# facebookresearch/co-tracker

Hardware: NVIDIA H100
Metric: tracked points*frames/sec at N=6400, T=16, 512^2 (higher is better)
Workload: dtype transformer + corr_mlp.fc2 + input_transform: bf16x3; correlation einsum: fp16x2; corr_mlp.fc1: bf16x3; fp32 accumulate, fp32 softmax/LayerNorm/GELU

## Files before the change

cotracker_b200/csrc/common.cuh:

```cuda
#pragma once
#include <cuda.h>
#include <cuda_bf16.h>
#include <cuda_fp16.h>
#include <cuda_runtime.h>
#include <stdint.h>

#include <atomic>

namespace ct3 {

struct DeviceOnce { std::atomic<uint64_t> done[2] = {}; };
template <typename F>
inline cudaError_t once_per_device(DeviceOnce& flag, F&& f) {
  int dev = 0;
  cudaError_t e = cudaGetDevice(&dev);
  if (e != cudaSuccess) return e;
  if (dev < 0 || dev >= 128) return f();
  const uint64_t bit = 1ull << (dev & 63);
  if (flag.done[dev >> 6].load(std::memory_order_acquire) & bit) return cudaSuccess;
  e = f();
  if (e == cudaSuccess) flag.done[dev >> 6].fetch_or(bit, std::memory_order_release);
  return e;
}

// ... 148 lines not shown
__device__ __forceinline__ uint8_t* smem_align1024(uint8_t* raw) {
  return raw + ((1024u - (smem_u32(raw) & 1023u)) & 1023u);
}

__device__ __forceinline__ void tma_prefetch_desc(const CUtensorMap* m) {
  asm volatile("prefetch.tensormap [%0];" ::"l"(reinterpret_cast<uint64_t>(m)) : "memory");
}
__device__ __forceinline__ void tma_load_2d(void* smem_dst, const CUtensorMap* m, int c0, int c1,
                                            uint64_t* bar) {
  asm volatile(
      "cp.async.bulk.tensor.2d.shared::cluster.global.mbarrier::complete_tx::bytes [%0], [%1, {%3, %4}], [%2];"
      ::"r"(smem_u32(smem_dst)), "l"(reinterpret_cast<uint64_t>(m)), "r"(smem_u32(bar)), "r"(c0), "r"(c1)
      : "memory");
}

__device__ __forceinline__ void tma_load_4d(void* smem_dst, const CUtensorMap* m, int c0, int c1, int c2, int c3,
                                            uint64_t* bar) {
  asm volatile(
      "cp.async.bulk.tensor.4d.shared::cluster.global.mbarrier::complete_tx::bytes [%0], [%1, {%3, %4, %5, %6}], [%2];"
      ::"r"(smem_u32(smem_dst)), "l"(reinterpret_cast<uint64_t>(m)), "r"(smem_u32(bar)), "r"(c0), "r"(c1), "r"(c2),
      "r"(c3)
      : "memory");
}

__device__ __forceinline__ uint64_t l2_policy_evict_first() {
  uint64_t p;
  asm volatile("createpolicy.fractional.L2::evict_first.b64 %0, 1.0;" : "=l"(p));
  return p;
}
__device__ __forceinline__ uint64_t l2_policy_evict_last() {
  uint64_t p;
  asm volatile("createpolicy.fractional.L2::evict_last.b64 %0, 1.0;" : "=l"(p));
  return p;
}
__device__ __forceinline__ void tma_load_4d_hint(void* smem_dst, const CUtensorMap* m, int c0, int c1, int c2, int c3,
                                                 uint64_t* bar, uint64_t policy) {
  asm volatile(
      "cp.async.bulk.tensor.4d.shared::cluster.global.mbarrier::complete_tx::bytes.L2::cache_hint [%0], [%1, {%3, %4, %5, %6}], [%2], %7;"
      ::"r"(smem_u32(smem_dst)), "l"(reinterpret_cast<uint64_t>(m)), "r"(smem_u32(bar)), "r"(c0), "r"(c1), "r"(c2),
      "r"(c3), "l"(policy)
      : "memory");
}
__device__ __forceinline__ void tma_load_3d(void* smem_dst, const CUtensorMap* m, int c0, int c1, int c2, uint64_t* bar) {
  asm volatile(
      "cp.async.bulk.tensor.3d.shared::cluster.global.mbarrier::complete_tx::bytes [%0], [%1, {%3, %4, %5}], [%2];"
      ::"r"(smem_u32(smem_dst)), "l"(reinterpret_cast<uint64_t>(m)), "r"(smem_u32(bar)), "r"(c0), "r"(c1), "r"(c2)
      : "memory");
}
__device__ __forceinline__ void tma_store_3d(const CUtensorMap* m, int c0, int c1, int c2, const void* smem_src) {
  asm volatile("cp.async.bulk.tensor.3d.global.shared::cta.bulk_group [%0, {%2, %3, %4}], [%1];"
               ::"l"(reinterpret_cast<uint64_t>(m)), "r"(smem_u32(smem_src)), "r"(c0), "r"(c1), "r"(c2)
               : "memory");
}

__device__ __forceinline__ void bulk_store_s2g(void* gdst, const void* ssrc, uint32_t bytes) {
  asm volatile("cp.async.bulk.global.shared::cta.bulk_group [%0], [%1], %2;" ::"l"(gdst), "r"(smem_u32(ssrc)), "r"(bytes)
               : "memory");
}
__device__ __forceinline__ void bulk_store_s2g_hint(void* gdst, const void* ssrc, uint32_t bytes, uint64_t policy) {
  asm volatile("cp.async.bulk.global.shared::cta.bulk_group.L2::cache_hint [%0], [%1], %2, %3;" ::"l"(gdst),
               "r"(smem_u32(ssrc)), "r"(bytes), "l"(policy)
               : "memory");
}
__device__ __forceinline__ void bulk_commit() { asm volatile("cp.async.bulk.commit_group;" ::: "memory"); }
__device__ __forceinline__ void bulk_wait_read0() { asm volatile("cp.async.bulk.wait_group.read 0;" ::: "memory"); }
__device__ __forceinline__ void bulk_wait0() { asm volatile("cp.async.bulk.wait_group 0;" ::: "memory"); }

__device__ __forceinline__ uint64_t gmma_desc_sw128(uint32_t smem_addr) {
  uint64_t d = 0;
  d |= (uint64_t)((smem_addr & 0x3FFFFu) >> 4);
  d |= (uint64_t)1 << 16;
  d |= (uint64_t)(1024 >> 4) << 32;
  d |= (uint64_t)1 << 62;
  return d;
}
__device__ __forceinline__ void wgmma_fence() { asm volatile("wgmma.fence.sync.aligned;" ::: "memory"); }
__device__ __forceinline__ void wgmma_commit() { asm volatile("wgmma.commit_group.sync.aligned;" ::: "memory"); }
template <int R>
__device__ __forceinline__ void wgmma_wait0(float (&d)[R]) {
  asm volatile("wgmma.wait_group.sync.aligned 0;" ::: "memory");
#pragma unroll
  for (int i = 0; i < R; ++i) asm volatile("" : "+f"(d[i])::"memory");
}

__device__ __forceinline__ void wgmma_m64n64_bf16(float (&d)[32], uint64_t da, uint64_t db, uint32_t scale_d) {
  asm volatile(
      "{\n\t.reg .pred p;\n\tsetp.ne.b32 p, %34, 0;\n\t"
      "wgmma.mma_async.sync.aligned.m64n64k16.f32.bf16.bf16 "
      "{%0, %1, %2, %3, %4, %5, %6, %7, %8, %9, %10, %11, %12, %13, %14, %15, %16, %17, %18, %19, %20, %21, %22, %23, %24, %25, %26, %27, %28, %29, %30, %31}, %32, %33, p, 1, 1, 0, 0;\n\t}"
      : "+f"(d[0]), "+f"(d[1]), "+f"(d[2]), "+f"(d[3]), "+f"(d[4]), "+f"(d[5]), "+f"(d[6]), "+f"(d[7]), "+f"(d[8]), "+f"(d[9]), "+f"(d[10]), "+f"(d[11]), "+f"(d[12]), "+f"(d[13]), "+f"(d[14]), "+f"(d[15]), "+f"(d[16]), "+f"(d[17]), "+f"(d[18]), "+f"(d[19]), "+f"(d[20]), "+f"(d[21]), "+f"(d[22]), "+f"(d[23]), "+f"(d[24]), "+f"(d[25]), "+f"(d[26]), "+f"(d[27]), "+f"(d[28]), "+f"(d[29]), "+f"(d[30]), "+f"(d[31])
      : "l"(da), "l"(db), "r"(scale_d));
}
__device__ __forceinline__ void wgmma_m64n128_bf16(float (&d)[64], uint64_t da, uint64_t db, uint32_t scale_d) {
  asm volatile(
      "{\n\t.reg .pred p;\n\tsetp.ne.b32 p, %66, 0;\n\t"
      "wgmma.mma_async.sync.aligned.m64n128k16.f32.bf16.bf16 "
      "{%0, %1, %2, %3, %4, %5, %6, %7, %8, %9, %10, %11, %12, %13, %14, %15, %16, %17, %18, %19, %20, %21, %22, %23, %24, %25, %26, %27, %28, %29, %30, %31, %32, %33, %34, %35, %36, %37, %38, %39, %40, %41, %42, %43, %44, %45, %46, %47, %48, %49, %50, %51, %52, %53, %54, %55, %56, %57, %58, %59, %60, %61, %62, %63}, %64, %65, p, 1, 1, 0, 0;\n\t}"
      : "+f"(d[0]), "+f"(d[1]), "+f"(d[2]), "+f"(d[3]), "+f"(d[4]), "+f"(d[5]), "+f"(d[6]), "+f"(d[7]), "+f"(d[8]), "+f"(d[9]), "+f"(d[10]), "+f"(d[11]), "+f"(d[12]), "+f"(d[13]), "+f"(d[14]), "+f"(d[15]), "+f"(d[16]), "+f"(d[17]), "+f"(d[18]), "+f"(d[19]), "+f"(d[20]), "+f"(d[21]), "+f"(d[22]), "+f"(d[23]), "+f"(d[24]), "+f"(d[25]), "+f"(d[26]), "+f"(d[27]), "+f"(d[28]), "+f"(d[29]), "+f"(d[30]), "+f"(d[31]), "+f"(d[32]), "+f"(d[33]), "+f"(d[34]), "+f"(d[35]), "+f"(d[36]), "+f"(d[37]), "+f"(d[38]), "+f"(d[39]), "+f"(d[40]), "+f"(d[41]), "+f"(d[42]), "+f"(d[43]), "+f"(d[44]), "+f"(d[45]), "+f"(d[46]), "+f"(d[47]), "+f"(d[48]), "+f"(d[49]), "+f"(d[50]), "+f"(d[51]), "+f"(d[52]), "+f"(d[53]), "+f"(d[54]), "+f"(d[55]), "+f"(d[56]), "+f"(d[57]), "+f"(d[58]), "+f"(d[59]), "+f"(d[60]), "+f"(d[61]), "+f"(d[62]), "+f"(d[63])
      : "l"(da), "l"(db), "r"(scale_d));
}
__device__ __forceinline__ void wgmma_m64n144_bf16(float (&d)[72], uint64_t da, uint64_t db, uint32_t scale_d) {
  asm volatile(
      "{\n\t.reg .pred p;\n\tsetp.ne.b32 p, %74, 0;\n\t"
      "wgmma.mma_async.sync.aligned.m64n144k16.f32.bf16.bf16 "
      "{%0, %1, %2, %3, %4, %5, %6, %7, %8, %9, %10, %11, %12, %13, %14, %15, %16, %17, %18, %19, %20, %21, %22, %23, %24, %25, %26, %27, %28, %29, %30, %31, %32, %33, %34, %35, %36, %37, %38, %39, %40, %41, %42, %43, %44, %45, %46, %47, %48, %49, %50, %51, %52, %53, %54, %55, %56, %57, %58, %59, %60, %61, %62, %63, %64, %65, %66, %67, %68, %69, %70, %71}, %72, %73, p, 1, 1, 0, 0;\n\t}"
      : "+f"(d[0]), "+f"(d[1]), "+f"(d[2]), "+f"(d[3]), "+f"(d[4]), "+f"(d[5]), "+f"(d[6]), "+f"(d[7]), "+f"(d[8]), "+f"(d[9]), "+f"(d[10]), "+f"(d[11]), "+f"(d[12]), "+f"(d[13]), "+f"(d[14]), "+f"(d[15]), "+f"(d[16]), "+f"(d[17]), "+f"(d[18]), "+f"(d[19]), "+f"(d[20]), "+f"(d[21]), "+f"(d[22]), "+f"(d[23]), "+f"(d[24]), "+f"(d[25]), "+f"(d[26]), "+f"(d[27]), "+f"(d[28]), "+f"(d[29]), "+f"(d[30]), "+f"(d[31]), "+f"(d[32]), "+f"(d[33]), "+f"(d[34]), "+f"(d[35]), "+f"(d[36]), "+f"(d[37]), "+f"(d[38]), "+f"(d[39]), "+f"(d[40]), "+f"(d[41]), "+f"(d[42]), "+f"(d[43]), "+f"(d[44]), "+f"(d[45]), "+f"(d[46]), "+f"(d[47]), "+f"(d[48]), "+f"(d[49]), "+f"(d[50]), "+f"(d[51]), "+f"(d[52]), "+f"(d[53]), "+f"(d[54]), "+f"(d[55]), "+f"(d[56]), "+f"(d[57]), "+f"(d[58]), "+f"(d[59]), "+f"(d[60]), "+f"(d[61]), "+f"(d[62]), "+f"(d[63]), "+f"(d[64]), "+f"(d[65]), "+f"(d[66]), "+f"(d[67]), "+f"(d[68]), "+f"(d[69]), "+f"(d[70]), "+f"(d[71])
      : "l"(da), "l"(db), "r"(scale_d));
}
__device__ __forceinline__ void wgmma_m64n64_f16(float (&d)[32], uint64_t da, uint64_t db, uint32_t scale_d) {
  asm volatile(
      "{\n\t.reg .pred p;\n\tsetp.ne.b32 p, %34, 0;\n\t"
      "wgmma.mma_async.sync.aligned.m64n64k16.f32.f16.f16 "
      "{%0, %1, %2, %3, %4, %5, %6, %7, %8, %9, %10, %11, %12, %13, %14, %15, %16, %17, %18, %19, %20, %21, %22, %23, %24, %25, %26, %27, %28, %29, %30, %31}, %32, %33, p, 1, 1, 0, 0;\n\t}"
      : "+f"(d[0]), "+f"(d[1]), "+f"(d[2]), "+f"(d[3]), "+f"(d[4]), "+f"(d[5]), "+f"(d[6]), "+f"(d[7]), "+f"(d[8]), "+f"(d[9]), "+f"(d[10]), "+f"(d[11]), "+f"(d[12]), "+f"(d[13]), "+f"(d[14]), "+f"(d[15]), "+f"(d[16]), "+f"(d[17]), "+f"(d[18]), "+f"(d[19]), "+f"(d[20]), "+f"(d[21]), "+f"(d[22]), "+f"(d[23]), "+f"(d[24]), "+f"(d[25]), "+f"(d[26]), "+f"(d[27]), "+f"(d[28]), "+f"(d[29]), "+f"(d[30]), "+f"(d[31])
      : "l"(da), "l"(db), "r"(scale_d));
}
__device__ __forceinline__ void wgmma_m64n128_f16(float (&d)[64], uint64_t da, uint64_t db, uint32_t scale_d) {
  asm volatile(
      "{\n\t.reg .pred p;\n\tsetp.ne.b32 p, %66, 0;\n\t"
      "wgmma.mma_async.sync.aligned.m64n128k16.f32.f16.f16 "
      "{%0, %1, %2, %3, %4, %5, %6, %7, %8, %9, %10, %11, %12, %13, %14, %15, %16, %17, %18, %19, %20, %21, %22, %23, %24, %25, %26, %27, %28, %29, %30, %31, %32, %33, %34, %35, %36, %37, %38, %39, %40, %41, %42, %43, %44, %45, %46, %47, %48, %49, %50, %51, %52, %53, %54, %55, %56, %57, %58, %59, %60, %61, %62, %63}, %64, %65, p, 1, 1, 0, 0;\n\t}"
      : "+f"(d[0]), "+f"(d[1]), "+f"(d[2]), "+f"(d[3]), "+f"(d[4]), "+f"(d[5]), "+f"(d[6]), "+f"(d[7]), "+f"(d[8]), "+f"(d[9]), "+f"(d[10]), "+f"(d[11]), "+f"(d[12]), "+f"(d[13]), "+f"(d[14]), "+f"(d[15]), "+f"(d[16]), "+f"(d[17]), "+f"(d[18]), "+f"(d[19]), "+f"(d[20]), "+f"(d[21]), "+f"(d[22]), "+f"(d[23]), "+f"(d[24]), "+f"(d[25]), "+f"(d[26]), "+f"(d[27]), "+f"(d[28]), "+f"(d[29]), "+f"(d[30]), "+f"(d[31]), "+f"(d[32]), "+f"(d[33]), "+f"(d[34]), "+f"(d[35]), "+f"(d[36]), "+f"(d[37]), "+f"(d[38]), "+f"(d[39]), "+f"(d[40]), "+f"(d[41]), "+f"(d[42]), "+f"(d[43]), "+f"(d[44]), "+f"(d[45]), "+f"(d[46]), "+f"(d[47]), "+f"(d[48]), "+f"(d[49]), "+f"(d[50]), "+f"(d[51]), "+f"(d[52]), "+f"(d[53]), "+f"(d[54]), "+f"(d[55]), "+f"(d[56]), "+f"(d[57]), "+f"(d[58]), "+f"(d[59]), "+f"(d[60]), "+f"(d[61]), "+f"(d[62]), "+f"(d[63])
      : "l"(da), "l"(db), "r"(scale_d));
}
__device__ __forceinline__ void wgmma_m64n144_f16(float (&d)[72], uint64_t da, uint64_t db, uint32_t scale_d) {
  asm volatile(
      "{\n\t.reg .pred p;\n\tsetp.ne.b32 p, %74, 0;\n\t"
      "wgmma.mma_async.sync.aligned.m64n144k16.f32.f16.f16 "
      "{%0, %1, %2, %3, %4, %5, %6, %7, %8, %9, %10, %11, %12, %13, %14, %15, %16, %17, %18, %19, %20, %21, %22, %23, %24, %25, %26, %27, %28, %29, %30, %31, %32, %33, %34, %35, %36, %37, %38, %39, %40, %41, %42, %43, %44, %45, %46, %47, %48, %49, %50, %51, %52, %53, %54, %55, %56, %57, %58, %59, %60, %61, %62, %63, %64, %65, %66, %67, %68, %69, %70, %71}, %72, %73, p, 1, 1, 0, 0;\n\t}"
      : "+f"(d[0]), "+f"(d[1]), "+f"(d[2]), "+f"(d[3]), "+f"(d[4]), "+f"(d[5]), "+f"(d[6]), "+f"(d[7]), "+f"(d[8]), "+f"(d[9]), "+f"(d[10]), "+f"(d[11]), "+f"(d[12]), "+f"(d[13]), "+f"(d[14]), "+f"(d[15]), "+f"(d[16]), "+f"(d[17]), "+f"(d[18]), "+f"(d[19]), "+f"(d[20]), "+f"(d[21]), "+f"(d[22]), "+f"(d[23]), "+f"(d[24]), "+f"(d[25]), "+f"(d[26]), "+f"(d[27]), "+f"(d[28]), "+f"(d[29]), "+f"(d[30]), "+f"(d[31]), "+f"(d[32]), "+f"(d[33]), "+f"(d[34]), "+f"(d[35]), "+f"(d[36]), "+f"(d[37]), "+f"(d[38]), "+f"(d[39]), "+f"(d[40]), "+f"(d[41]), "+f"(d[42]), "+f"(d[43]), "+f"(d[44]), "+f"(d[45]), "+f"(d[46]), "+f"(d[47]), "+f"(d[48]), "+f"(d[49]), "+f"(d[50]), "+f"(d[51]), "+f"(d[52]), "+f"(d[53]), "+f"(d[54]), "+f"(d[55]), "+f"(d[56]), "+f"(d[57]), "+f"(d[58]), "+f"(d[59]), "+f"(d[60]), "+f"(d[61]), "+f"(d[62]), "+f"(d[63]), "+f"(d[64]), "+f"(d[65]), "+f"(d[66]), "+f"(d[67]), "+f"(d[68]), "+f"(d[69]), "+f"(d[70]), "+f"(d[71])
      : "l"(da), "l"(db), "r"(scale_d));
}

__device__ __forceinline__ void wgmma_m64n48_bf16(float (&d)[24], uint64_t da, uint64_t db, uint32_t scale_d) {
  asm volatile(
      "{\n\t.reg .pred p;\n\tsetp.ne.b32 p, %26, 0;\n\t"
      "wgmma.mma_async.sync.aligned.m64n48k16.f32.bf16.bf16 "
      "{%0, %1, %2, %3, %4, %5, %6, %7, %8, %9, %10, %11, %12, %13, %14, %15, %16, %17, %18, %19, %20, %21, %22, %23}, %24, %25, p, 1, 1, 0, 0;\n\t}"
      : "+f"(d[0]), "+f"(d[1]), "+f"(d[2]), "+f"(d[3]), "+f"(d[4]), "+f"(d[5]), "+f"(d[6]), "+f"(d[7]), "+f"(d[8]), "+f"(d[9]), "+f"(d[10]), "+f"(d[11]), "+f"(d[12]), "+f"(d[13]), "+f"(d[14]), "+f"(d[15]), "+f"(d[16]), "+f"(d[17]), "+f"(d[18]), "+f"(d[19]), "+f"(d[20]), "+f"(d[21]), "+f"(d[22]), "+f"(d[23])
      : "l"(da), "l"(db), "r"(scale_d));
}
__device__ __forceinline__ void wgmma_m64n64_bf16_head(float (&d)[64], uint64_t da, uint64_t db, uint32_t scale_d) {
  asm volatile(
      "{\n\t.reg .pred p;\n\tsetp.ne.b32 p, %34, 0;\n\t"
      "wgmma.mma_async.sync.aligned.m64n64k16.f32.bf16.bf16 "
      "{%0, %1, %2, %3, %4, %5, %6, %7, %8, %9, %10, %11, %12, %13, %14, %15, %16, %17, %18, %19, %20, %21, %22, %23, %24, %25, %26, %27, %28, %29, %30, %31}, %32, %33, p, 1, 1, 0, 0;\n\t}"
      : "+f"(d[0]), "+f"(d[1]), "+f"(d[2]), "+f"(d[3]), "+f"(d[4]), "+f"(d[5]), "+f"(d[6]), "+f"(d[7]), "+f"(d[8]), "+f"(d[9]), "+f"(d[10]), "+f"(d[11]), "+f"(d[12]), "+f"(d[13]), "+f"(d[14]), "+f"(d[15]), "+f"(d[16]), "+f"(d[17]), "+f"(d[18]), "+f"(d[19]), "+f"(d[20]), "+f"(d[21]), "+f"(d[22]), "+f"(d[23]), "+f"(d[24]), "+f"(d[25]), "+f"(d[26]), "+f"(d[27]), "+f"(d[28]), "+f"(d[29]), "+f"(d[30]), "+f"(d[31])
      : "l"(da), "l"(db), "r"(scale_d));
}
__device__ __forceinline__ void wgmma_m64n64_f16_head(float (&d)[64], uint64_t da, uint64_t db, uint32_t scale_d) {
  asm volatile(
      "{\n\t.reg .pred p;\n\tsetp.ne.b32 p, %34, 0;\n\t"
      "wgmma.mma_async.sync.aligned.m64n64k16.f32.f16.f16 "
      "{%0, %1, %2, %3, %4, %5, %6, %7, %8, %9, %10, %11, %12, %13, %14, %15, %16, %17, %18, %19, %20, %21, %22, %23, %24, %25, %26, %27, %28, %29, %30, %31}, %32, %33, p, 1, 1, 0, 0;\n\t}"
      : "+f"(d[0]), "+f"(d[1]), "+f"(d[2]), "+f"(d[3]), "+f"(d[4]), "+f"(d[5]), "+f"(d[6]), "+f"(d[7]), "+f"(d[8]), "+f"(d[9]), "+f"(d[10]), "+f"(d[11]), "+f"(d[12]), "+f"(d[13]), "+f"(d[14]), "+f"(d[15]), "+f"(d[16]), "+f"(d[17]), "+f"(d[18]), "+f"(d[19]), "+f"(d[20]), "+f"(d[21]), "+f"(d[22]), "+f"(d[23]), "+f"(d[24]), "+f"(d[25]), "+f"(d[26]), "+f"(d[27]), "+f"(d[28]), "+f"(d[29]), "+f"(d[30]), "+f"(d[31])
      : "l"(da), "l"(db), "r"(scale_d));
}
template <int N, bool F16>
__device__ __forceinline__ void wgmma_tile(float (&d)[N / 2], uint64_t da, uint64_t db, uint32_t scale_d) {
  if constexpr (N == 48) {
    static_assert(!F16, "wgmma_tile: N = 48 is bf16 only");
    wgmma_m64n48_bf16(d, da, db, scale_d);
  } else if constexpr (N == 64) {
    if constexpr (F16) wgmma_m64n64_f16(d, da, db, scale_d); else wgmma_m64n64_bf16(d, da, db, scale_d);
  } else if constexpr (N == 128) {
    if constexpr (F16) wgmma_m64n128_f16(d, da, db, scale_d); else wgmma_m64n128_bf16(d, da, db, scale_d);
// ... 61 lines not shown
```

cotracker_b200/csrc/gemm.cu:

```cuda
#include "gemm.cuh"

namespace ct3 {
namespace {

constexpr int BM = 128, BN = 128, BK = 64;
constexpr int TILE_A = BM * BK * 2;
constexpr int TILE_B = BN * BK * 2;
constexpr int MMA_WARPS = 4;
constexpr int TMA_WARP = 4;
constexpr int EPI_WARP0 = 8;
constexpr int EPI_WARPS = 8;
constexpr int CW = 16;
constexpr int STG_WORDS = 32 * CW;
constexpr int MAX_STAGES = 4;
template <int NPROD>
struct Cfg {
  static constexpr int AP = NPROD >= 3 ? 2 : 1;
  static constexpr int BP = NPROD >= 2 ? 2 : 1;
  static constexpr int STAGE_BYTES = AP * TILE_A + BP * TILE_B;
  static constexpr int STAGES = NPROD >= 2 ? 2 : 4;
  static constexpr int OFF_B = AP * TILE_A;
};
constexpr int RING_BYTES = 2 * 65536;
static_assert(Cfg<1>::STAGES * Cfg<1>::STAGE_BYTES <= RING_BYTES && Cfg<2>::STAGES * Cfg<2>::STAGE_BYTES <= RING_BYTES &&
              Cfg<3>::STAGES * Cfg<3>::STAGE_BYTES <= RING_BYTES, "ring size");
constexpr int ACC_LD = BN + 4;
constexpr int OFF_ACC = RING_BYTES;
constexpr int OFF_STG = OFF_ACC + BM * ACC_LD * 4;
constexpr int OFF_BAR = OFF_STG + EPI_WARPS * STG_WORDS * 4;
constexpr int SMEM_BYTES = OFF_BAR + 256  + 1024 ;
static_assert(SMEM_BYTES <= 232448, "shared memory budget");
constexpr int THREADS = (EPI_WARP0 + EPI_WARPS) * 32;
constexpr int REG_TMA = 40, REG_MMA = 216, REG_EPI = 65536 / THREADS;
static_assert(128 * (REG_TMA + REG_MMA + 2 * REG_EPI) <= 65536, "register budget");

__device__ __forceinline__ float apply_act(float x, int act) {
  if (act == 1) return gelu_erf(x);
  if (act == 2) return gelu_tanh(x);
  return x;
}

__device__ __forceinline__ int stg_idx(int row, int word) { return row * CW + ((word + (row >> 1)) & (CW - 1)); }

__device__ __forceinline__ void epilogue_chunk(const GemmEpilogue& e, int M, int N, int row0, int col0, int lane,
                                               float (&v)[CW], uint32_t* stg) {
  const int row = row0 + lane;
  if (e.bias) {
    const float4* b4 = reinterpret_cast<const float4*>(e.bias + col0);
#pragma unroll
    for (int i = 0; i < CW / 4; ++i) {
      float4 b = __ldg(b4 + i);
      v[4 * i + 0] += b.x; v[4 * i + 1] += b.y; v[4 * i + 2] += b.z; v[4 * i + 3] += b.w;
    }
  }
  if (e.row_bias && row < M) {
    const float4* b4 = reinterpret_cast<const float4*>(e.row_bias + (int64_t)(row % e.row_mod) * N + col0);
#pragma unroll
    for (int i = 0; i < CW / 4; ++i) {
      float4 b = __ldg(b4 + i);
      v[4 * i + 0] += b.x; v[4 * i + 1] += b.y; v[4 * i + 2] += b.z; v[4 * i + 3] += b.w;
    }
  }
  if (e.act != 0) {
#pragma unroll
    for (int i = 0; i < CW; ++i) v[i] = apply_act(v[i], e.act);
  }
  const int rsub = lane >> 2, q = lane & 3;
  if (e.out_f32) {
#pragma unroll
    for (int c = 0; c < CW; ++c) stg[stg_idx(lane, c)] = __float_as_uint(v[c]);
    __syncwarp();
    float* base = e.out_f32 + (int64_t)(row0 + rsub) * e.ld_f32 + col0 + 4 * q;
    const int64_t rstep = 8 * e.ld_f32;
    float4 x[4];
#pragma unroll
    for (int k = 0; k < 4; ++k) {
      const int r = 8 * k + rsub;
      x[k] = make_float4(__uint_as_float(stg[stg_idx(r, 4 * q + 0)]), __uint_as_float(stg[stg_idx(r, 4 * q + 1)]),
                         __uint_as_float(stg[stg_idx(r, 4 * q + 2)]), __uint_as_float(stg[stg_idx(r, 4 * q + 3)]));
    }
    if (e.residual) {
      float4 r4[4];
#pragma unroll
      for (int k = 0; k < 4; ++k)
        r4[k] = (row0 + 8 * k + rsub < M) ? *reinterpret_cast<const float4*>(base + k * rstep) : make_float4(0.f, 0.f, 0.f, 0.f);
#pragma unroll
      for (int k = 0; k < 4; ++k) { x[k].x += r4[k].x; x[k].y += r4[k].y; x[k].z += r4[k].z; x[k].w += r4[k].w; }
    }
#pragma unroll
    for (int k = 0; k < 4; ++k)
      if (row0 + 8 * k + rsub < M) *reinterpret_cast<float4*>(base + k * rstep) = x[k];
    __syncwarp();
  }
  if (e.out_split) {
#pragma unroll
    for (int i = 0; i < CW / 2; ++i) {
      uint32_t hi, lo;
      split2(v[2 * i], v[2 * i + 1], hi, lo);
      stg[stg_idx(lane, i)] = hi;
      stg[stg_idx(lane, CW / 2 + i)] = lo;
    }
    __syncwarp();
    uint32_t off16_lane = 0xffffffffu;
    if (row < M) {
      const int orow = row / e.row_group;
      off16_lane = (uint32_t)(((long long)orow * e.ld_split + (long long)(row % e.row_group) * N + col0) >> 3);
    }
    uint4* plane = reinterpret_cast<uint4*>(e.out_split + (q >= 2 ? e.lo_off : 0)) + (q & 1);
#pragma unroll
    for (int k = 0; k < 4; ++k) {
      const int r = 8 * k + rsub;
      const uint32_t o16 = __shfl_sync(0xffffffffu, off16_lane, r);
      const uint4 w4 = make_uint4(stg[stg_idx(r, 4 * q + 0)], stg[stg_idx(r, 4 * q + 1)], stg[stg_idx(r, 4 * q + 2)],
                                  stg[stg_idx(r, 4 * q + 3)]);
      if (o16 != 0xffffffffu) plane[o16] = w4;
    }
    __syncwarp();
  }
}

template <int NPROD>
__global__ void __launch_bounds__(THREADS, 1)
gemm_split3_tc_kernel(const __grid_constant__ CUtensorMap tmX, const __grid_constant__ CUtensorMap tmW, int M,
                      int N, int Kpad, int fp16, GemmEpilogue epi) {
  using C = Cfg<NPROD>;
  constexpr int STAGES = C::STAGES, STAGE_BYTES = C::STAGE_BYTES;
  extern __shared__ __align__(1024) uint8_t smem_raw[];
  uint8_t* smem = smem_align1024(smem_raw);
  uint64_t* full_bar = reinterpret_cast<uint64_t*>(smem + OFF_BAR);
  uint64_t* empty_bar = full_bar + MAX_STAGES;
  uint64_t* tfull_bar = empty_bar + MAX_STAGES;
  uint64_t* tempty_bar = tfull_bar + 1;
  float* acc_tile = reinterpret_cast<float*>(smem + OFF_ACC);

  const int warp = threadIdx.x >> 5, lane = threadIdx.x & 31;

  if (threadIdx.x == 0) {
    tma_prefetch_desc(&tmX);
    tma_prefetch_desc(&tmW);
    for (int i = 0; i < STAGES; ++i) {
      mbar_init(&full_bar[i], 1);
      mbar_init(&empty_bar[i], MMA_WARPS);
    }
    mbar_init(tfull_bar, MMA_WARPS);
    mbar_init(tempty_bar, EPI_WARPS * 32);
    fence_barrier_init();
  }
  __syncthreads();

  const int num_mt = (M + BM - 1) / BM;
  const int num_nt = N / BN;
  const int num_tiles = num_mt * num_nt;
  const int num_kb = Kpad / BK;

  if (warp >= MMA_WARPS && warp < EPI_WARP0) {
    setmaxnreg_dec<REG_TMA>();
    if (warp == TMA_WARP && elect_one()) {
      int stage = 0;
      uint32_t phase = 0;
      for (int tile = blockIdx.x; tile < num_tiles; tile += gridDim.x) {
        const int mt = tile / num_nt, nt = tile % num_nt;
        for (int kb = 0; kb < num_kb; ++kb) {
          mbar_wait(&empty_bar[stage], phase ^ 1u);
          mbar_arrive_expect_tx(&full_bar[stage], STAGE_BYTES);
          uint8_t* s = smem + stage * STAGE_BYTES;
          tma_load_2d(s, &tmX, kb * BK, mt * BM, &full_bar[stage]);
          if (C::AP == 2) tma_load_2d(s + TILE_A, &tmX, Kpad + kb * BK, mt * BM, &full_bar[stage]);
          tma_load_2d(s + C::OFF_B, &tmW, kb * BK, nt * BN, &full_bar[stage]);
          if (C::BP == 2) tma_load_2d(s + C::OFF_B + TILE_B, &tmW, Kpad + kb * BK, nt * BN, &full_bar[stage]);
          if (++stage == STAGES) { stage = 0; phase ^= 1u; }
        }
      }
    }
  } else if (warp < MMA_WARPS) {
    setmaxnreg_inc<REG_MMA>();
    int stage = 0;
    uint32_t phase = 0, acc_phase = 0;
    for (int tile = blockIdx.x; tile < num_tiles; tile += gridDim.x) {
      float d0[BN / 2], d1[BN / 2];
      for (int kb = 0; kb < num_kb; ++kb) {
        mbar_wait(&full_bar[stage], phase);
        wgmma_fence();
        const uint32_t sa = smem_u32(smem + stage * STAGE_BYTES);
        if (fp16) mma_kblock<NPROD, BN, true>(d0, d1, sa, TILE_A, C::OFF_B, TILE_B, kb == 0);
        else mma_kblock<NPROD, BN, false>(d0, d1, sa, TILE_A, C::OFF_B, TILE_B, kb == 0);
        wgmma_commit();
        wgmma_wait0(d0);
        wgmma_wait0(d1);
        __syncwarp();
        if (lane == 0) mbar_arrive(&empty_bar[stage]);
        if (++stage == STAGES) { stage = 0; phase ^= 1u; }
      }
      mbar_wait(tempty_bar, acc_phase ^ 1u);
      acc_store<BN>(d0, acc_tile, ACC_LD);
      acc_store<BN>(d1, acc_tile + 64 * ACC_LD, ACC_LD);
      __syncwarp();
      if (lane == 0) mbar_arrive(tfull_bar);
      acc_phase ^= 1u;
    }
  } else {
    const int e = warp - EPI_WARP0;
    const int quarter = e & 3;
    constexpr int CH = BN / CW / (EPI_WARPS / 4);
    const int chunk0 = (e >> 2) * CH;
    uint32_t acc_phase = 0;
    for (int tile = blockIdx.x; tile < num_tiles; tile += gridDim.x) {
      const int mt = tile / num_nt, nt = tile % num_nt;
      mbar_wait(tfull_bar, acc_phase);
      const int row0 = mt * BM + quarter * 32;
      uint32_t* stg = reinterpret_cast<uint32_t*>(smem + OFF_STG) + e * STG_WORDS;
      const float* arow = acc_tile + (quarter * 32 + lane) * ACC_LD;
#pragma unroll 1
      for (int chunk = chunk0; chunk < chunk0 + CH; ++chunk) {
        float v[CW];
        acc_row_ld<CW>(arow + chunk * CW, v);
        epilogue_chunk(epi, M, N, row0, nt * BN + chunk * CW, lane, v, stg);
      }
      mbar_arrive(tempty_bar);
      acc_phase ^= 1u;
    }
  }
}

namespace qa {
constexpr int BNQ = 144;
constexpr int TILE_BQ = BNQ * BK * 2;
constexpr int STAGE = 2 * TILE_A + 2 * TILE_BQ;
constexpr int NSTAGE = 2;
constexpr int QACC_LD = BNQ + 4;
constexpr int QOFF_ACC = NSTAGE * STAGE;
constexpr int OFF_BARQ = QOFF_ACC + BM * QACC_LD * 4;
constexpr int SMEM = OFF_BARQ + 256 + 1024;
constexpr int EPIW = 4;
constexpr int QEPI_WARP0 = 8;
constexpr int NTHREADS = 12 * 32;
constexpr int REG_PRODUCER = 40, REG_COMPUTE = 232;
static_assert(128 * (REG_PRODUCER + 2 * REG_COMPUTE) <= NTHREADS * 168, "register budget");
static_assert(SMEM <= 232448, "shared memory budget");
}

__global__ void __launch_bounds__(qa::NTHREADS, 1)
gemm_qkv_time_attn_kernel(const __grid_constant__ CUtensorMap tmX, const __grid_constant__ CUtensorMap tmW, int M,
                          int Kpad, int T, int R, float scale_log2e, GemmEpilogue epi) {
  using namespace qa;
  extern __shared__ __align__(1024) uint8_t smem_raw[];
  uint8_t* smem = smem_align1024(smem_raw);
  uint64_t* full_bar = reinterpret_cast<uint64_t*>(smem + OFF_BARQ);
  uint64_t* empty_bar = full_bar + NSTAGE;
  uint64_t* tfull_bar = empty_bar + NSTAGE;
  uint64_t* tempty_bar = tfull_bar + 1;
  float* acc = reinterpret_cast<float*>(smem + QOFF_ACC);

  const int warp = threadIdx.x >> 5, lane = threadIdx.x & 31;
  if (threadIdx.x == 0) {
    tma_prefetch_desc(&tmX);
    tma_prefetch_desc(&tmW);
    for (int i = 0; i < NSTAGE; ++i) {
      mbar_init(&full_bar[i], 1);
      mbar_init(&empty_bar[i], MMA_WARPS);
    }
    mbar_init(tfull_bar, MMA_WARPS);
    mbar_init(tempty_bar, EPIW * 32);
    fence_barrier_init();
  }
  __syncthreads();

  const int num_mt = (M + R - 1) / R;
  const int num_tiles = num_mt * kHeads;
  const int num_kb = Kpad / BK;

  if (warp >= MMA_WARPS && warp < QEPI_WARP0) {
    setmaxnreg_dec<REG_PRODUCER>();
    if (warp == TMA_WARP && elect_one()) {
      int stage = 0;
      uint32_t phase = 0;
      for (int tile = blockIdx.x; tile < num_tiles; tile += gridDim.x) {
        const int mt = tile / kHeads, h = tile % kHeads;
        for (int kb = 0; kb < num_kb; ++kb) {
          mbar_wait(&empty_bar[stage], phase ^ 1u);
          mbar_arrive_expect_tx(&full_bar[stage], STAGE);
          uint8_t* s = smem + stage * STAGE;
          tma_load_2d(s, &tmX, kb * BK, mt * R, &full_bar[stage]);
          tma_load_2d(s + TILE_A, &tmX, Kpad + kb * BK, mt * R, &full_bar[stage]);
          tma_load_2d(s + 2 * TILE_A, &tmW, kb * BK, h * BNQ, &full_bar[stage]);
          tma_load_2d(s + 2 * TILE_A + TILE_BQ, &tmW, Kpad + kb * BK, h * BNQ, &full_bar[stage]);
          if (++stage == NSTAGE) { stage = 0; phase ^= 1u; }
        }
      }
    }
  } else if (warp < MMA_WARPS) {
    setmaxnreg_inc<REG_COMPUTE>();
    int stage = 0;
    uint32_t phase = 0, acc_phase = 0;
    for (int tile = blockIdx.x; tile < num_tiles; tile += gridDim.x) {
      float d0[BNQ / 2], d1[BNQ / 2];
      for (int kb = 0; kb < num_kb; ++kb) {
        mbar_wait(&full_bar[stage], phase);
        wgmma_fence();
        mma_kblock<3, BNQ, false>(d0, d1, smem_u32(smem + stage * STAGE), TILE_A, 2 * TILE_A, TILE_BQ, kb == 0);
        wgmma_commit();
        wgmma_wait0(d0);
        wgmma_wait0(d1);
// ... 140 lines not shown
  __shared__ float Bs[16][64 + 1];
  const int tx = threadIdx.x & 15, ty = threadIdx.x >> 4;
  const int m0 = blockIdx.y * 64, n0 = blockIdx.x * 64;
  float acc[4][4] = {};
  const int64_t ld = 2 * (int64_t)Kpad;
  auto val = [fp16](const __nv_bfloat16* p) {
    return fp16 ? __half2float(*reinterpret_cast<const __half*>(p)) : __bfloat162float(*p);
  };
  for (int k0 = 0; k0 < Kpad; k0 += 16) {
    for (int i = threadIdx.x; i < 64 * 16; i += 256) {
      const int r = i >> 4, k = i & 15;
      const int gm = m0 + r, gn = n0 + r;
      float a = 0.f, b = 0.f;
      if (gm < M) a = val(X + gm * x_ld + k0 + k) + (products == 3 ? val(X + gm * x_ld + Kpad + k0 + k) : 0.f);
      if (gn < N) b = val(W + gn * ld + k0 + k) + (products >= 2 ? val(W + gn * ld + Kpad + k0 + k) : 0.f);
      As[k][r] = a;
      Bs[k][r] = b;
    }
    __syncthreads();
#pragma unroll
    for (int k = 0; k < 16; ++k) {
      float a[4], b[4];
#pragma unroll
      for (int i = 0; i < 4; ++i) { a[i] = As[k][ty * 4 + i]; b[i] = Bs[k][tx * 4 + i]; }
#pragma unroll
      for (int i = 0; i < 4; ++i)
#pragma unroll
        for (int j = 0; j < 4; ++j) acc[i][j] = fmaf(a[i], b[j], acc[i][j]);
    }
    __syncthreads();
  }
  for (int i = 0; i < 4; ++i)
    for (int j = 0; j < 4; ++j) {
      const int r = m0 + ty * 4 + i, c = n0 + tx * 4 + j;
      if (r < M && c < N) epilogue_store1(epi, N, r, c, acc[i][j]);
    }
}

typedef CUresult (*EncodeTiledFn)(CUtensorMap*, CUtensorMapDataType, cuuint32_t, void*, const cuuint64_t*,
                                  const cuuint64_t*, const cuuint32_t*, const cuuint32_t*, CUtensorMapInterleave,
                                  CUtensorMapSwizzle, CUtensorMapL2promotion, CUtensorMapFloatOOBfill);

EncodeTiledFn get_encode_fn() {
  static const EncodeTiledFn fn = [] {
    void* p = nullptr;
    cudaDriverEntryPointQueryResult q;
    if (cudaGetDriverEntryPoint("cuTensorMapEncodeTiled", &p, cudaEnableDefault, &q) == cudaSuccess &&
        q == cudaDriverEntryPointSuccess)
      return reinterpret_cast<EncodeTiledFn>(p);
    return (EncodeTiledFn) nullptr;
  }();
  return fn;
}

bool make_tmap(CUtensorMap* m, const void* base, uint64_t rows, uint64_t cols, uint32_t box_rows = 128) {
  EncodeTiledFn fn = get_encode_fn();
  if (!fn) return false;
  cuuint64_t dims[2] = {cols, rows};
  cuuint64_t strides[1] = {cols * 2};
  cuuint32_t box[2] = {64, box_rows};
  cuuint32_t estr[2] = {1, 1};
  CUresult r = fn(m, CU_TENSOR_MAP_DATA_TYPE_BFLOAT16, 2, const_cast<void*>(base), dims, strides, box, estr,
                  CU_TENSOR_MAP_INTERLEAVE_NONE, CU_TENSOR_MAP_SWIZZLE_128B, CU_TENSOR_MAP_L2_PROMOTION_L2_128B,
                  CU_TENSOR_MAP_FLOAT_OOB_FILL_NONE);
  return r == CUDA_SUCCESS;
}

}

bool encode_tensor_map(CUtensorMap* m, CUtensorMapDataType dtype, int rank, const void* base, const uint64_t* dims,
                       const uint64_t* strides_bytes, const uint32_t* box, CUtensorMapSwizzle swizzle) {
  EncodeTiledFn fn = get_encode_fn();
  if (!fn || rank < 1 || rank > 5) return false;
  cuuint64_t d[5], st[5];
  cuuint32_t b[5], es[5];
  for (int i = 0; i < rank; ++i) { d[i] = dims[i]; b[i] = box[i]; es[i] = 1; }
  for (int i = 0; i + 1 < rank; ++i) st[i] = strides_bytes[i];
  return fn(m, dtype, (cuuint32_t)rank, const_cast<void*>(base), d, st, b, es, CU_TENSOR_MAP_INTERLEAVE_NONE, swizzle,
            CU_TENSOR_MAP_L2_PROMOTION_L2_256B, CU_TENSOR_MAP_FLOAT_OOB_FILL_NONE) == CUDA_SUCCESS;
}

namespace {

template <int NPROD>
cudaError_t launch_tc(const GemmProblem& p, const CUtensorMap& tmX, const CUtensorMap& tmW, int num_mt, int num_sms,
                      cudaStream_t stream) {
  static DeviceOnce attr;
  cudaError_t e = once_per_device(attr, [&] {
    return cudaFuncSetAttribute(gemm_split3_tc_kernel<NPROD>, cudaFuncAttributeMaxDynamicSharedMemorySize, SMEM_BYTES);
  });
  if (e != cudaSuccess) return e;
  const int num_tiles = num_mt * (p.N / BN);
  const int grid = num_tiles < num_sms ? num_tiles : num_sms;
  gemm_split3_tc_kernel<NPROD><<<grid, THREADS, SMEM_BYTES, stream>>>(tmX, tmW, p.M, p.N, p.Kpad, p.fp16, p.epi);
  return cudaGetLastError();
}

}

bool qkv_time_attn_supported(int T) { return T >= 1 && T <= BM; }

int gemm_qkv_time_attn_launch(const __nv_bfloat16* x_split, const __nv_bfloat16* w_heads, const float* bias_heads,
                              int M, int Kpad, int T, __nv_bfloat16* att_split, int64_t ld_split, int lo_off,
                              float scale, int num_sms, cudaStream_t stream, const char** err) {
  *err = nullptr;
  if (M <= 0 || Kpad <= 0 || (Kpad % BK) != 0 || !qkv_time_attn_supported(T) || (M % T) != 0) {
    *err = "qkv_time_attn: need M > 0, M % T == 0, 1 <= T <= 128, Kpad % 64 == 0";
    return (int)cudaErrorInvalidValue;
  }
  if (((reinterpret_cast<uintptr_t>(x_split) | reinterpret_cast<uintptr_t>(w_heads) |
        reinterpret_cast<uintptr_t>(att_split)) & 15) || (ld_split % 8) != 0 || (lo_off % 8) != 0) {
    *err = "qkv_time_attn: operands must be 16-byte aligned";
    return (int)cudaErrorInvalidValue;
  }
  const int R = (BM / T) * T;
  CUtensorMap tmX, tmW;
  if (!make_tmap(&tmX, x_split, (uint64_t)M, 2ull * Kpad) ||
      !make_tmap(&tmW, w_heads, (uint64_t)(kHeads * qa::BNQ), 2ull * Kpad, (uint32_t)qa::BNQ)) {
    *err = "qkv_time_attn: cuTensorMapEncodeTiled failed";
    return (int)cudaErrorInvalidValue;
  }
  static DeviceOnce attr;
  cudaError_t e = once_per_device(attr, [&] {
    return cudaFuncSetAttribute(gemm_qkv_time_attn_kernel, cudaFuncAttributeMaxDynamicSharedMemorySize, qa::SMEM);
  });
  if (e != cudaSuccess) { *err = "qkv_time_attn: cudaFuncSetAttribute failed"; return (int)e; }
  const int num_tiles = ((M + R - 1) / R) * kHeads;
  GemmEpilogue epi;
  epi.bias = bias_heads;
  epi.out_split = att_split;
  epi.ld_split = ld_split;
  epi.lo_off = lo_off;
  gemm_qkv_time_attn_kernel<<<num_tiles < num_sms ? num_tiles : num_sms, qa::NTHREADS, qa::SMEM, stream>>>(
      tmX, tmW, M, Kpad, T, R, scale * 1.44269504088896340736f, epi);
  return (int)cudaGetLastError();
}

const char* gemm_check(const GemmProblem& p) {
  if (p.M <= 0 || p.N <= 0 || p.Kpad <= 0 || (p.N % BN) != 0 || (p.Kpad % BK) != 0)
    return "gemm: need M>0, N % 128 == 0, Kpad % 64 == 0";
  if (p.products < 1 || p.products > 3 || p.fp16 < 0 || p.fp16 > 1) return "gemm: products in 1..3, fp16 in 0..1";
  const int64_t x_ld = p.x_ld ? p.x_ld : 2 * (int64_t)p.Kpad;
  if (x_ld < (p.products == 3 ? 2 : 1) * (int64_t)p.Kpad || (x_ld % 8) != 0)
    return "gemm: x_ld too small for the operand planes this product count reads";
  if ((reinterpret_cast<uintptr_t>(p.x_split) | reinterpret_cast<uintptr_t>(p.w_split)) & 15)
    return "gemm: operands must be 16-byte aligned";
  const GemmEpilogue& e = p.epi;
  if (!e.out_f32 && !e.out_split) return "gemm: no output";
  if (e.row_mod < 1 || e.row_group < 1 || e.act < 0 || e.act > 2) return "gemm: need row_mod >= 1, row_group >= 1, act in 0..2";
  if (e.out_f32 && (e.ld_f32 < p.N || (e.ld_f32 % 4) != 0)) return "gemm: fp32 output pitch must be >= N and a multiple of 4";
  if (e.out_split) {
    const int64_t width = (int64_t)e.row_group * p.N;
    if ((e.ld_split % 8) != 0 || (e.lo_off % 8) != 0) return "gemm: split output pitch and lo offset must be multiples of 8";
    if (e.lo_off < width || e.ld_split < e.lo_off + width) return "gemm: hi and lo planes of the split output overlap";
  }
  if ((reinterpret_cast<uintptr_t>(e.bias) | reinterpret_cast<uintptr_t>(e.row_bias) |
       reinterpret_cast<uintptr_t>(e.out_f32) | reinterpret_cast<uintptr_t>(e.out_split)) & 15)
    return "gemm: bias, row bias and outputs must be 16-byte aligned";
  return nullptr;
}

int gemm_launch(const GemmProblem& p, int impl, int num_sms, cudaStream_t stream, const char** err) {
  *err = gemm_check(p);
  if (*err) return (int)cudaErrorInvalidValue;
  const int64_t x_ld = p.x_ld ? p.x_ld : 2 * (int64_t)p.Kpad;
  if (impl == 1) {
    dim3 grid((p.N + 63) / 64, (p.M + 63) / 64);
    gemm_split3_simt_kernel<<<grid, 256, 0, stream>>>(p.x_split, p.w_split, p.M, p.N, p.Kpad, x_ld, p.products,
                                                      p.fp16, p.epi);
    return (int)cudaGetLastError();
  }
  const int num_mt = (p.M + BM - 1) / BM;
  CUtensorMap tmX, tmW;
  if (!make_tmap(&tmX, p.x_split, (uint64_t)p.M, (uint64_t)x_ld) ||
      !make_tmap(&tmW, p.w_split, (uint64_t)p.N, 2ull * p.Kpad)) {
    *err = "gemm: cuTensorMapEncodeTiled failed";
    return (int)cudaErrorInvalidValue;
  }
// ... 8 lines not shown
```

Baseline: 632,600.

## Add half-tile accumulator handoff with deeper ring for long-K split GEMMs

For GEMMs with at least 16 K-blocks, the MMA warps hand the accumulator to the epilogue in two 64-row halves. This lets the next tile's first K-block start while the epilogue drains, and keeps one wgmma group in flight (wait_group 1) before releasing stages. The freed accumulator space and the removed per-warp staging buffer are spent on a 3x64KB ring, giving 3-6 stages instead of 2-4. The epilogue now stages its transposes in the accumulator tile rows. This adds complexity in barrier phase handling and in the template variants.

```diff
diff --git a/cotracker_b200/csrc/common.cuh b/cotracker_b200/csrc/common.cuh
--- a/cotracker_b200/csrc/common.cuh
+++ b/cotracker_b200/csrc/common.cuh
@@ -254,6 +254,12 @@
 #pragma unroll
   for (int i = 0; i < R; ++i) asm volatile("" : "+f"(d[i])::"memory");
 }
+template <int R>
+__device__ __forceinline__ void wgmma_wait1(float (&d0)[R], float (&d1)[R]) {
+  asm volatile("wgmma.wait_group.sync.aligned 1;" ::: "memory");
+#pragma unroll
+  for (int i = 0; i < R; ++i) asm volatile("" : "+f"(d0[i]), "+f"(d1[i])::"memory");
+}
 
 __device__ __forceinline__ void wgmma_m64n64_bf16(float (&d)[32], uint64_t da, uint64_t db, uint32_t scale_d) {
   asm volatile(
diff --git a/cotracker_b200/csrc/gemm.cu b/cotracker_b200/csrc/gemm.cu
--- a/cotracker_b200/csrc/gemm.cu
+++ b/cotracker_b200/csrc/gemm.cu
@@ -11,25 +11,29 @@
 constexpr int EPI_WARP0 = 8;
 constexpr int EPI_WARPS = 8;
 constexpr int CW = 16;
-constexpr int STG_WORDS = 32 * CW;
-constexpr int MAX_STAGES = 4;
-template <int NPROD>
+constexpr int ACC_LD = BN + 4;
+constexpr int MAX_STAGES = 6;
+constexpr int BAR_BYTES = 256;
+constexpr int HALVES_MIN_KB = 16;
+static_assert((2 * MAX_STAGES + 2) * 8 <= BAR_BYTES, "barriers");
+template <int NPROD, bool HALVES>
 struct Cfg {
   static constexpr int AP = NPROD >= 3 ? 2 : 1;
   static constexpr int BP = NPROD >= 2 ? 2 : 1;
   static constexpr int STAGE_BYTES = AP * TILE_A + BP * TILE_B;
-  static constexpr int STAGES = NPROD >= 2 ? 2 : 4;
   static constexpr int OFF_B = AP * TILE_A;
+  static constexpr int RING_BYTES = (HALVES ? 3 : 2) * 65536;
+  static constexpr int STAGES = RING_BYTES / STAGE_BYTES;
+  static constexpr int HAND_M = HALVES ? BM / 2 : BM;
+  static constexpr int OFF_ACC = RING_BYTES;
+  static constexpr int OFF_BAR = OFF_ACC + HAND_M * ACC_LD * 4;
+  static constexpr int SMEM_BYTES = OFF_BAR + BAR_BYTES + 1024 ;
+  static_assert(STAGES <= MAX_STAGES && SMEM_BYTES <= 232448, "shared memory budget");
 };
-constexpr int RING_BYTES = 2 * 65536;
-static_assert(Cfg<1>::STAGES * Cfg<1>::STAGE_BYTES <= RING_BYTES && Cfg<2>::STAGES * Cfg<2>::STAGE_BYTES <= RING_BYTES &&
-              Cfg<3>::STAGES * Cfg<3>::STAGE_BYTES <= RING_BYTES, "ring size");
-constexpr int ACC_LD = BN + 4;
-constexpr int OFF_ACC = RING_BYTES;
-constexpr int OFF_STG = OFF_ACC + BM * ACC_LD * 4;
-constexpr int OFF_BAR = OFF_STG + EPI_WARPS * STG_WORDS * 4;
-constexpr int SMEM_BYTES = OFF_BAR + 256  + 1024 ;
-static_assert(SMEM_BYTES <= 232448, "shared memory budget");
+static_assert(Cfg<3, false>::STAGES == 2 && Cfg<2, false>::STAGES == 2 && Cfg<1, false>::STAGES == 4, "ring depth");
+static_assert(Cfg<3, true>::STAGES == 3 && Cfg<2, true>::STAGES == 4 && Cfg<1, true>::STAGES == 6, "ring depth");
+static_assert(Cfg<3, false>::SMEM_BYTES == 131072 + 67584 + 1280 && Cfg<3, true>::SMEM_BYTES == 196608 + 33792 + 1280,
+              "shared memory layout");
 constexpr int THREADS = (EPI_WARP0 + EPI_WARPS) * 32;
 constexpr int REG_TMA = 40, REG_MMA = 216, REG_EPI = 65536 / THREADS;
 static_assert(128 * (REG_TMA + REG_MMA + 2 * REG_EPI) <= 65536, "register budget");
@@ -40,10 +44,8 @@
   return x;
 }
 
-__device__ __forceinline__ int stg_idx(int row, int word) { return row * CW + ((word + (row >> 1)) & (CW - 1)); }
-
 __device__ __forceinline__ void epilogue_chunk(const GemmEpilogue& e, int M, int N, int row0, int col0, int lane,
-                                               float (&v)[CW], uint32_t* stg) {
+                                               float (&v)[CW], float* c) {
   const int row = row0 + lane;
   if (e.bias) {
     const float4* b4 = reinterpret_cast<const float4*>(e.bias + col0);
@@ -65,20 +67,18 @@
 #pragma unroll
     for (int i = 0; i < CW; ++i) v[i] = apply_act(v[i], e.act);
   }
-  const int rsub = lane >> 2, q = lane & 3;
+  const int rsub = (lane >> 3) + 4 * ((lane >> 2) & 1), q = lane & 3;
+  float4* mine = reinterpret_cast<float4*>(c + lane * ACC_LD);
+  auto staged = [&](int k) { return reinterpret_cast<const float4*>(c + (8 * k + rsub) * ACC_LD) + q; };
   if (e.out_f32) {
 #pragma unroll
-    for (int c = 0; c < CW; ++c) stg[stg_idx(lane, c)] = __float_as_uint(v[c]);
+    for (int i = 0; i < CW / 4; ++i) mine[i] = make_float4(v[4 * i], v[4 * i + 1], v[4 * i + 2], v[4 * i + 3]);
     __syncwarp();
     float* base = e.out_f32 + (int64_t)(row0 + rsub) * e.ld_f32 + col0 + 4 * q;
     const int64_t rstep = 8 * e.ld_f32;
     float4 x[4];
 #pragma unroll
-    for (int k = 0; k < 4; ++k) {
-      const int r = 8 * k + rsub;
-      x[k] = make_float4(__uint_as_float(stg[stg_idx(r, 4 * q + 0)]), __uint_as_float(stg[stg_idx(r, 4 * q + 1)]),
-                         __uint_as_float(stg[stg_idx(r, 4 * q + 2)]), __uint_as_float(stg[stg_idx(r, 4 * q + 3)]));
-    }
+    for (int k = 0; k < 4; ++k) x[k] = *staged(k);
     if (e.residual) {
       float4 r4[4];
 #pragma unroll
@@ -93,13 +93,14 @@
     __syncwarp();
   }
   if (e.out_split) {
-#pragma unroll
-    for (int i = 0; i < CW / 2; ++i) {
-      uint32_t hi, lo;
-      split2(v[2 * i], v[2 * i + 1], hi, lo);
-      stg[stg_idx(lane, i)] = hi;
-      stg[stg_idx(lane, CW / 2 + i)] = lo;
-    }
+    uint32_t hi[CW / 2], lo[CW / 2];
+#pragma unroll
+    for (int i = 0; i < CW / 2; ++i) split2(v[2 * i], v[2 * i + 1], hi[i], lo[i]);
+    uint4* mine4 = reinterpret_cast<uint4*>(mine);
+    mine4[0] = make_uint4(hi[0], hi[1], hi[2], hi[3]);
+    mine4[1] = make_uint4(hi[4], hi[5], hi[6], hi[7]);
+    mine4[2] = make_uint4(lo[0], lo[1], lo[2], lo[3]);
+    mine4[3] = make_uint4(lo[4], lo[5], lo[6], lo[7]);
     __syncwarp();
     uint32_t off16_lane = 0xffffffffu;
     if (row < M) {
@@ -109,29 +110,90 @@
     uint4* plane = reinterpret_cast<uint4*>(e.out_split + (q >= 2 ? e.lo_off : 0)) + (q & 1);
 #pragma unroll
     for (int k = 0; k < 4; ++k) {
-      const int r = 8 * k + rsub;
-      const uint32_t o16 = __shfl_sync(0xffffffffu, off16_lane, r);
-      const uint4 w4 = make_uint4(stg[stg_idx(r, 4 * q + 0)], stg[stg_idx(r, 4 * q + 1)], stg[stg_idx(r, 4 * q + 2)],
-                                  stg[stg_idx(r, 4 * q + 3)]);
+      const uint32_t o16 = __shfl_sync(0xffffffffu, off16_lane, 8 * k + rsub);
+      const uint4 w4 = *reinterpret_cast<const uint4*>(staged(k));
       if (o16 != 0xffffffffu) plane[o16] = w4;
     }
     __syncwarp();
   }
 }
 
-template <int NPROD>
+template <int NPROD, bool F16, int HALF>
+__device__ __forceinline__ void mma_kblock0_half(float (&d)[BN / 2], uint32_t s) {
+  using C = Cfg<NPROD, true>;
+  const uint32_t a_hi = s + HALF * (TILE_A / 2), a_lo = a_hi + TILE_A, b_hi = s + C::OFF_B, b_lo = b_hi + TILE_B;
+#pragma unroll
+  for (int kk = 0; kk < 4; ++kk)
+    mma_k16<NPROD, BN, F16>(d, a_hi + kk * 32, a_lo + kk * 32, b_hi + kk * 32, b_lo + kk * 32, kk == 0 ? 0u : 1u);
+}
+
+template <int NPROD, bool F16>
+__device__ __forceinline__ void mma_half_tiles(uint8_t* smem, uint64_t* full_bar, uint64_t* empty_bar,
+                                               uint64_t* tfull_bar, uint64_t* tempty_bar, int num_tiles, int num_kb) {
+  using C = Cfg<NPROD, true>;
+  float* acc_tile = reinterpret_cast<float*>(smem + C::OFF_ACC);
+  const int lane = threadIdx.x & 31;
+  int stage = 0, held = 0;
+  uint32_t phase = 0, acc_phase = 0;
+  float d0[BN / 2], d1[BN / 2];
+  auto release_held = [&] {
+    __syncwarp();
+    if (lane == 0) mbar_arrive(&empty_bar[held]);
+  };
+  auto advance = [&] {
+    held = stage;
+    if (++stage == C::STAGES) { stage = 0; phase ^= 1u; }
+  };
+  auto hand_off = [&](const float (&d)[BN / 2]) {
+    mbar_wait(tempty_bar, acc_phase ^ 1u);
+    acc_store<BN>(d, acc_tile, ACC_LD);
+    __syncwarp();
+    if (lane == 0) mbar_arrive(tfull_bar);
+    acc_phase ^= 1u;
+  };
+  if (blockIdx.x >= num_tiles) return;
+  for (int tile = blockIdx.x, kb_first = 0;; tile += gridDim.x, kb_first = 1) {
+    for (int kb = kb_first; kb < num_kb; ++kb) {
+      mbar_wait(&full_bar[stage], phase);
+      wgmma_fence();
+      mma_kblock<NPROD, BN, F16>(d0, d1, smem_u32(smem + stage * C::STAGE_BYTES), TILE_A, C::OFF_B, TILE_B, kb == 0);
+      wgmma_commit();
+      wgmma_wait1(d0, d1);
+      if (kb > 0) release_held();
+      advance();
+    }
+    wgmma_wait0(d0);
+    wgmma_wait0(d1);
+    release_held();
+    hand_off(d0);
+    if (tile + (int)gridDim.x >= num_tiles) break;
+    const uint32_t sa = smem_u32(smem + stage * C::STAGE_BYTES);
+    mbar_wait(&full_bar[stage], phase);
+    wgmma_fence();
+    mma_kblock0_half<NPROD, F16, 0>(d0, sa);
+    wgmma_commit();
+    hand_off(d1);
+    wgmma_fence();
+    mma_kblock0_half<NPROD, F16, 1>(d1, sa);
+    wgmma_commit();
+    advance();
+  }
+  hand_off(d1);
+}
+
+template <int NPROD, bool HALVES>
 __global__ void __launch_bounds__(THREADS, 1)
 gemm_split3_tc_kernel(const __grid_constant__ CUtensorMap tmX, const __grid_constant__ CUtensorMap tmW, int M,
                       int N, int Kpad, int fp16, GemmEpilogue epi) {
-  using C = Cfg<NPROD>;
+  using C = Cfg<NPROD, HALVES>;
   constexpr int STAGES = C::STAGES, STAGE_BYTES = C::STAGE_BYTES;
   extern __shared__ __align__(1024) uint8_t smem_raw[];
   uint8_t* smem = smem_align1024(smem_raw);
-  uint64_t* full_bar = reinterpret_cast<uint64_t*>(smem + OFF_BAR);
+  uint64_t* full_bar = reinterpret_cast<uint64_t*>(smem + C::OFF_BAR);
   uint64_t* empty_bar = full_bar + MAX_STAGES;
   uint64_t* tfull_bar = empty_bar + MAX_STAGES;
   uint64_t* tempty_bar = tfull_bar + 1;
-  float* acc_tile = reinterpret_cast<float*>(smem + OFF_ACC);
+  float* acc_tile = reinterpret_cast<float*>(smem + C::OFF_ACC);
 
   const int warp = threadIdx.x >> 5, lane = threadIdx.x & 31;
 
@@ -174,50 +236,58 @@
     }
   } else if (warp < MMA_WARPS) {
     setmaxnreg_inc<REG_MMA>();
-    int stage = 0;
-    uint32_t phase = 0, acc_phase = 0;
-    for (int tile = blockIdx.x; tile < num_tiles; tile += gridDim.x) {
-      float d0[BN / 2], d1[BN / 2];
-      for (int kb = 0; kb < num_kb; ++kb) {
-        mbar_wait(&full_bar[stage], phase);
-        wgmma_fence();
-        const uint32_t sa = smem_u32(smem + stage * STAGE_BYTES);
-        if (fp16) mma_kblock<NPROD, BN, true>(d0, d1, sa, TILE_A, C::OFF_B, TILE_B, kb == 0);
-        else mma_kblock<NPROD, BN, false>(d0, d1, sa, TILE_A, C::OFF_B, TILE_B, kb == 0);
-        wgmma_commit();
-        wgmma_wait0(d0);
-        wgmma_wait0(d1);
+    if constexpr (HALVES) {
+      if (fp16) mma_half_tiles<NPROD, true>(smem, full_bar, empty_bar, tfull_bar, tempty_bar, num_tiles, num_kb);
+      else mma_half_tiles<NPROD, false>(smem, full_bar, empty_bar, tfull_bar, tempty_bar, num_tiles, num_kb);
+    } else {
+      int stage = 0;
+      uint32_t phase = 0, acc_phase = 0;
+      for (int tile = blockIdx.x; tile < num_tiles; tile += gridDim.x) {
+        float d0[BN / 2], d1[BN / 2];
+        for (int kb = 0; kb < num_kb; ++kb) {
+          mbar_wait(&full_bar[stage], phase);
+          wgmma_fence();
+          const uint32_t sa = smem_u32(smem + stage * STAGE_BYTES);
+          if (fp16) mma_kblock<NPROD, BN, true>(d0, d1, sa, TILE_A, C::OFF_B, TILE_B, kb == 0);
+          else mma_kblock<NPROD, BN, false>(d0, d1, sa, TILE_A, C::OFF_B, TILE_B, kb == 0);
+          wgmma_commit();
+          wgmma_wait0(d0);
+          wgmma_wait0(d1);
+          __syncwarp();
+          if (lane == 0) mbar_arrive(&empty_bar[stage]);
+          if (++stage == STAGES) { stage = 0; phase ^= 1u; }
+        }
+        mbar_wait(tempty_bar, acc_phase ^ 1u);
+        acc_store<BN>(d0, acc_tile, ACC_LD);
+        acc_store<BN>(d1, acc_tile + 64 * ACC_LD, ACC_LD);
         __syncwarp();
-        if (lane == 0) mbar_arrive(&empty_bar[stage]);
-        if (++stage == STAGES) { stage = 0; phase ^= 1u; }
+        if (lane == 0) mbar_arrive(tfull_bar);
+        acc_phase ^= 1u;
       }
-      mbar_wait(tempty_bar, acc_phase ^ 1u);
-      acc_store<BN>(d0, acc_tile, ACC_LD);
-      acc_store<BN>(d1, acc_tile + 64 * ACC_LD, ACC_LD);
-      __syncwarp();
-      if (lane == 0) mbar_arrive(tfull_bar);
-      acc_phase ^= 1u;
     }
   } else {
+    constexpr int RG = C::HAND_M / 32;
+    constexpr int CH = BN / CW / (EPI_WARPS / RG);
     const int e = warp - EPI_WARP0;
-    const int quarter = e & 3;
-    constexpr int CH = BN / CW / (EPI_WARPS / 4);
-    const int chunk0 = (e >> 2) * CH;
+    const int rg = e % RG;
+    const int chunk0 = (e / RG) * CH;
+    float* const group = acc_tile + rg * 32 * ACC_LD;
     uint32_t acc_phase = 0;
     for (int tile = blockIdx.x; tile < num_tiles; tile += gridDim.x) {
       const int mt = tile / num_nt, nt = tile % num_nt;
-      mbar_wait(tfull_bar, acc_phase);
-      const int row0 = mt * BM + quarter * 32;
-      uint32_t* stg = reinterpret_cast<uint32_t*>(smem + OFF_STG) + e * STG_WORDS;
-      const float* arow = acc_tile + (quarter * 32 + lane) * ACC_LD;
 #pragma unroll 1
-      for (int chunk = chunk0; chunk < chunk0 + CH; ++chunk) {
-        float v[CW];
-        acc_row_ld<CW>(arow + chunk * CW, v);
-        epilogue_chunk(epi, M, N, row0, nt * BN + chunk * CW, lane, v, stg);
+      for (int h = 0; h < BM / C::HAND_M; ++h) {
+        mbar_wait(tfull_bar, acc_phase);
+        const int row0 = mt * BM + h * C::HAND_M + rg * 32;
+#pragma unroll 1
+        for (int chunk = chunk0; chunk < chunk0 + CH; ++chunk) {
+          float v[CW];
+          acc_row_ld<CW>(group + lane * ACC_LD + chunk * CW, v);
+          epilogue_chunk(epi, M, N, row0, nt * BN + chunk * CW, lane, v, group + chunk * CW);
+        }
+        mbar_arrive(tempty_bar);
+        acc_phase ^= 1u;
       }
-      mbar_arrive(tempty_bar);
-      acc_phase ^= 1u;
     }
   }
 }
@@ -524,18 +594,26 @@
 
 namespace {
 
-template <int NPROD>
-cudaError_t launch_tc(const GemmProblem& p, const CUtensorMap& tmX, const CUtensorMap& tmW, int num_mt, int num_sms,
-                      cudaStream_t stream) {
+template <int NPROD, bool HALVES>
+cudaError_t launch_tc_layout(const GemmProblem& p, const CUtensorMap& tmX, const CUtensorMap& tmW, int num_mt,
+                             int num_sms, cudaStream_t stream) {
+  constexpr int smem = Cfg<NPROD, HALVES>::SMEM_BYTES;
   static DeviceOnce attr;
   cudaError_t e = once_per_device(attr, [&] {
-    return cudaFuncSetAttribute(gemm_split3_tc_kernel<NPROD>, cudaFuncAttributeMaxDynamicSharedMemorySize, SMEM_BYTES);
+    return cudaFuncSetAttribute(gemm_split3_tc_kernel<NPROD, HALVES>, cudaFuncAttributeMaxDynamicSharedMemorySize, smem);
   });
   if (e != cudaSuccess) return e;
   const int num_tiles = num_mt * (p.N / BN);
   const int grid = num_tiles < num_sms ? num_tiles : num_sms;
-  gemm_split3_tc_kernel<NPROD><<<grid, THREADS, SMEM_BYTES, stream>>>(tmX, tmW, p.M, p.N, p.Kpad, p.fp16, p.epi);
+  gemm_split3_tc_kernel<NPROD, HALVES><<<grid, THREADS, smem, stream>>>(tmX, tmW, p.M, p.N, p.Kpad, p.fp16, p.epi);
   return cudaGetLastError();
+}
+
+template <int NPROD>
+cudaError_t launch_tc(const GemmProblem& p, const CUtensorMap& tmX, const CUtensorMap& tmW, int num_mt, int num_sms,
+                      cudaStream_t stream) {
+  return p.Kpad / BK >= HALVES_MIN_KB ? launch_tc_layout<NPROD, true>(p, tmX, tmW, num_mt, num_sms, stream)
+                                      : launch_tc_layout<NPROD, false>(p, tmX, tmW, num_mt, num_sms, stream);
 }
 
 }
```

Measured after the change: 644,600, median of 6. 1.02x the previous value.
